# idiap/ilqr_planner

Measured on AMD Instinct MI355X. Metric: iLQR iterations/sec (7-DoF, T=200, batch 4096) + final-cost rel-err vs Eigen ref, higher is better.
Workload: dtype f64; 1 GPU; C3: PosOrn nb_deriv=1 7-DoF Panda chain, T=200, batch 4096/GPU x 1 GPU = 4096, solver=al, 20 iterations/solve, line search on, early stop off; global_batch=4096, horizon=200, parallelism=instances sharded x1, exchange=none

## Files before the change

ilqr_planner_amd/capi.py:

```python
from __future__ import annotations

import collections
import ctypes as C
import os

import numpy as np

_HERE = os.path.dirname(os.path.abspath(__file__))
LIB_PATH = os.path.join(_HERE, "libilqr_hip.so")

MAX_SEG, MAX_KP, MAX_NX, MAX_NU, MAX_NF, MAX_NQ = 24, 8, 15, 8, 15, 13
SYS_POS_ORN, SYS_POS_ORN_TIME, SYS_JOINT, SYS_JOINT_TIME = 0, 1, 2, 3
STATUS_OK, STATUS_NONFINITE, STATUS_ALPHA_FLOOR, STATUS_SWEEP_IO = 0, 1, 2, 4
LQT_MAX_NX, LQT_MAX_NU = 16, 8
CL_STATS = 5
KP_ERR, KP_STATS, CL_OUTCOME = 5, 12, 4
CL_CON_STATS, CL_OUTCOME_CON = 6, 5
KP_ERR_POS, KP_ERR_ORN, KP_ERR_VEL, KP_ERR_ANGVEL, KP_ERR_TIME = range(5)
PROF_ROLLOUT, PROF_BACKWARD, PROF_FORWARD, PROF_OTHER, PROF_APPLY = 0, 1, 2, 3, 4

EXPORTS = [
    "ilqr_dims_of", "ilqr_desc_defaults", "ilqr_ctx_create", "ilqr_ctx_destroy", "ilqr_last_error", "ilqr_ctx_set_stream",
    "ilqr_ctx_synchronize", "ilqr_version", "ilqr_problem_create", "ilqr_problem_destroy", "ilqr_problem_set_init_state",
    "ilqr_problem_set_keypoint_targets", "ilqr_problem_set_controls", "ilqr_problem_set_constraints",
# ... 282 lines not shown
        self._problems = weakref.WeakSet()
        rc = self.L.ilqr_ctx_create(device_id, C.byref(self.h))
        if rc:
            raise RuntimeError(f"ilqr_ctx_create failed (code {rc}): no usable HIP device {device_id}; there is no CPU fallback")

    def check(self, rc):
        if rc:
            raise RuntimeError(self.L.ilqr_last_error(self.h).decode())

    def set_stream(self, stream_ptr):
        self.check(self.L.ilqr_ctx_set_stream(self.h, C.c_void_p(stream_ptr)))

    def synchronize(self):
        self.check(self.L.ilqr_ctx_synchronize(self.h))

    _PINS = {"sweep": {None: 0, "mfma": 1, "rows": 2, "siwave": 4, "siwg": 5, "siwgio": 6}, "forward": {None: 0, "wg": 1, "dpp": 2, "wglds": 3}, "reroll": {None: 0, "rows": 1, "dpp": 2}}

    def set_crosscheck(self, generic_kernels=False, cp_lane_solve=False, cp_general=False, sweep=None, forward=None, reroll=None):
        pins = []
        for name, v in (("sweep", sweep), ("forward", forward), ("reroll", reroll)):
            if v not in self._PINS[name]:
                raise ValueError(f"set_crosscheck: {name} must be one of {[k for k in self._PINS[name] if k]} or None (got {v!r})")
            pins.append(self._PINS[name][v])
        self.check(self.L.ilqr_ctx_set_crosscheck(self.h, int(bool(generic_kernels)), int(bool(cp_lane_solve)), int(bool(cp_general)), *pins))

    def crosscheck_from_env(self):
        env = os.environ
        self.set_crosscheck(env.get("ILQR_HIP_PATH") == "v1", env.get("ILQR_CP_SOLVE") == "lane", env.get("ILQR_CP") == "general",
                            sweep=env.get("ILQR_SWEEP") or None, forward=env.get("ILQR_FWD") or None, reroll=env.get("ILQR_APPLY") or None)

    def set_split(self, mode: int):
# ... 433 lines not shown
```

ilqr_planner_amd/csrc/ilqr_capi.cpp:

```cpp
#include "../../include/ilqr_hip.h"

#include <hip/hip_runtime.h>

#include <cmath>
#include <cstdio>
#include <cstdlib>
#include <cstring>
#include <string>
#include <vector>

#include "ilqr_batchcp.hpp"
#include "ilqr_closed_loop.hpp"
#include "ilqr_closed_loop_cov.hpp"
#include "ilqr_ctx.hpp"
#include "ilqr_kernels.hpp"
#include "ilqr_plan.hpp"

using namespace ilqr;

struct DevScratch {
    double* ptr = nullptr;
    size_t elems = 0;
    int reserve(ilqr_ctx* c, size_t n) {
        if (elems >= n) return 0;
// ... 111 lines not shown

extern "C" int ilqr_ctx_set_stream(ilqr_ctx* c, void* s) {
    if (!c) return 1;
    c->stream = s ? (hipStream_t)s : c->own_stream;
    return 0;
}

extern "C" int ilqr_ctx_set_split(ilqr_ctx* c, int on) {
    if (!c) return 1;
    if (on < 0 || on > 2) return fail(c, "ilqr_ctx_set_split: mode must be 0, 1 or 2 (got " + std::to_string(on) + ")");
    c->split = on;
    return 0;
}

static_assert((int)SweepPin::Mfma == ILQR_XC_SWEEP_MFMA && (int)SweepPin::Rows == ILQR_XC_SWEEP_ROWS && (int)SweepPin::SiWave == ILQR_XC_SWEEP_SI_WAVE &&
              (int)SweepPin::SiWg == ILQR_XC_SWEEP_SI_WG && (int)SweepPin::SiWgIo == ILQR_XC_SWEEP_SI_WG_IO && (int)FwdPin::Wg == ILQR_XC_FWD_WG &&
              (int)FwdPin::Dpp == ILQR_XC_FWD_DPP && (int)FwdPin::WgLds == ILQR_XC_FWD_WG_LDS && (int)RerollPin::Rows == ILQR_XC_REROLL_ROWS && (int)RerollPin::Dpp == ILQR_XC_REROLL_DPP,
              "variant pins of ilqr_plan.hpp and include/ilqr_hip.h");

extern "C" int ilqr_ctx_set_crosscheck(ilqr_ctx* c, int generic_kernels, int cp_lane_solve, int cp_general, int sweep, int forward, int reroll) {
    if (!c) return 1;
    if (sweep < 0 || sweep > 6 || sweep == 3) return fail(c, "ilqr_ctx_set_crosscheck: sweep must be ILQR_XC_AUTO, ILQR_XC_SWEEP_MFMA, ILQR_XC_SWEEP_ROWS, ILQR_XC_SWEEP_SI_WAVE, ILQR_XC_SWEEP_SI_WG or ILQR_XC_SWEEP_SI_WG_IO");
    if (forward < 0 || forward > 3) return fail(c, "ilqr_ctx_set_crosscheck: forward must be ILQR_XC_AUTO, ILQR_XC_FWD_WG, ILQR_XC_FWD_DPP or ILQR_XC_FWD_WG_LDS");
    if (reroll < 0 || reroll > 2) return fail(c, "ilqr_ctx_set_crosscheck: reroll must be ILQR_XC_AUTO, ILQR_XC_REROLL_ROWS or ILQR_XC_REROLL_DPP");
    c->xc_sweep = (SweepPin)sweep;
    c->xc_forward = (FwdPin)forward;
    c->xc_reroll = (RerollPin)reroll;
    c->xc_generic = generic_kernels != 0;
    c->xc_cp_lane = cp_lane_solve != 0;
    c->xc_cp_general = cp_general != 0;
    return 0;
}

extern "C" int ilqr_ctx_synchronize(ilqr_ctx* c) {
    if (!c) return 1;
    HIPCHK(c, hipStreamSynchronize(c->stream));
    return 0;
// ... 485 lines not shown
static FwdArgs plan_fwd_args(const ilqr_problem* p, const RiccatiPlan& pl) {
    FwdArgs f;
    std::memset(&f, 0, sizeof(f));
    f.n_alpha = pl.n_alpha; f.n_kp = p->hdesc.steps.n;
    f.shared = has_shared_step(p->hdesc.steps) ? 1 : 0;
    f.n_kp_all = p->desc.n_kp;
    f.fused = pl.fused ? 1 : 0;
    f.fwd_lds = pl.fwd_lds ? 1 : 0;
    f.limits = p->desc.limits_set ? 1 : 0;
    for (int k = 0; k < p->desc.n_kp; k++) f.kp_ext |= p->desc.kp_dist[k] | p->desc.kp_has_frame[k] | p->desc.kp_has_Ru[k] | p->desc.kp_joint[k];
    return f;
}
static void launch_sweep(const ilqr_problem* p, const RiccatiPlan& pl, int h, bool al, const Bufs& bf, int B, hipStream_t st, SweepArgs& sw) {
    const int kind = p->desc.kind, nd = p->desc.nb_deriv;
    switch (pl.sweep) {
        case Sweep::SiDpp: sw.si_wg = pl.si_wg[h] ? 1 : 0; sw.si_io = pl.si_io[h] ? 1 : 0; launch_backward_si_dpp(al, pl.fused, pl.kd_sym == 1, pl.si_lanes[h], bf, B, st, sw); break;
        case Sweep::Rows: launch_backward_rows(kind, nd, al, bf, B, st); break;
        case Sweep::Mfma: launch_backward_mfma(kind, nd, al, bf, B, st); break;
        case Sweep::Generic: launch_backward_generic(kind, nd, al, bf, B, st); break;
    }
}

static int solve_riccati(ilqr_problem* p, bool al, int nb_iter, int lag, double penalty0, double scaling, int line_search, int early_stop) {
    if (!p) return 1;
    ilqr_ctx* c = p->ctx;
    if (!p->has_state || !p->has_controls) return fail(c, "set_init_state and set_controls must be called before a solve");
    if (nb_iter < 0) return fail(c, "nb_iter < 0");
    if (al && (p->bufs.m <= 0 || lag <= 0)) return fail(c, "AL solve needs constraints (ilqr_problem_set_constraints) and lag_update_step > 0");
    HIPCHK(c, hipSetDevice(c->device));
    if (ensure_trace(p, nb_iter)) return 1;
    p->last_nb_iter = nb_iter;
// ... 11 lines not shown
    FwdArgs f = plan_fwd_args(p, pl);
    f.line_search = line_search; f.early_stop = early_stop; f.nb_iter = nb_iter; f.penalty_roll = penalty0; f.al = al ? 1 : 0;
    for (int h = 0; h < nh; h++) {
        const Bufs& bf = hv[h].bufs;
        ProfScope ps(c, ILQR_PROF_ROLLOUT);
        if (pl.init == Init::Lti) launch_init_lti(kind, nd, bf, hv[h].B, hv[h].st);
        else launch_init(kind, nd, al, bf, hv[h].B, hv[h].st, penalty0);
        if (pl.init_al_update) {
            f.it = -1; f.do_update = 0;
            launch_al_update(kind, nd, bf, hv[h].B, T, hv[h].st, f);
        }
    }
    HIPCHK(c, hipGetLastError());
    double penalty = penalty0;
    SweepArgs sw;
    sw.pen_in = penalty; sw.pen_update_prev = penalty; sw.do_update_prev = 0; sw.si_wg = 0; sw.si_io = 0;
    for (int it = 0; it < nb_iter; it++) {
        FwdArgs fi = f;
        fi.it = it;
        fi.penalty_roll = penalty;
        fi.do_update = al && ((it + 1) % lag == 0);
        if (fi.do_update) penalty *= scaling;
        fi.penalty_update = penalty;
        for (int h = 0; h < nh; h++) {
            const Bufs& bf = hv[h].bufs;
            const int B = hv[h].B;
            hipStream_t st = hv[h].st;
            if (pl.split && it == 0 && h == 1) HIPCHK(c, hipStreamWaitEvent(st, c->ev_stagger, 0));
            {
                ProfScope ps(c, ILQR_PROF_OTHER);
                launch_kp_derivs(kind, nd, bf, B, st, fi);
// ... 102 lines not shown
    if (!p->has_plan)
        return fail(c, "ilqr_problem_gains needs a plan: run a solver since the problem's inputs last changed (ilqr_solve_recursive with nb_iter = 0 rolls out the controls as they are)");
    HIPCHK(c, hipSetDevice(c->device));
    const int kind = p->desc.kind, nd = p->desc.nb_deriv;
    const RiccatiPlan pl = plan_riccati(plan_input(p, false, 1, 1));
    p->has_gains = false;
    p->bufs.kd_sym = pl.kd_sym;
    if (pl.needs_ws && !p->bufs.ws)
        if (dalloc(p, &p->bufs.ws, (size_t)backward_ws_entries(kind, nd) * p->Bp, false)) return 1;
    Half hv[2];
    int nh = 1;
    if (split_begin(p, pl.split, hv, nh)) return 1;
    SplitJoin split_join{c, pl.split};
    const FwdArgs f = plan_fwd_args(p, pl);
    SweepArgs sw;
    sw.pen_in = 0.0; sw.pen_update_prev = 0.0; sw.do_update_prev = 0; sw.si_wg = 0; sw.si_io = 0;
    for (int h = 0; h < nh; h++) {
        const Bufs& bf = hv[h].bufs;
        const int B = hv[h].B;
        hipStream_t st = hv[h].st;
        {
            ProfScope ps(c, ILQR_PROF_OTHER);
            launch_gains_prepare(bf, B, st);
        }
        {
            ProfScope ps(c, ILQR_PROF_OTHER);
            launch_kp_derivs(kind, nd, bf, B, st, f);
        }
        {
            ProfScope ps(c, ILQR_PROF_BACKWARD);
            launch_sweep(p, pl, h, false, bf, B, st, sw);
// ... 536 lines not shown
```

ilqr_planner_amd/csrc/ilqr_kernels.hpp:

```cpp
#pragma once
#include <hip/hip_runtime.h>

#include "ilqr_device.hpp"
#include "ilqr_dofmap.hpp"

namespace ilqr {

struct Bufs {
    const DevDesc* desc;
    double* X[2];
    double* U[2];
    const double* U0;
    double* KD;
    const double* q0;
    const double* dq0;
    const double* kp_tg;
    double* cost;
    double* alpha;
    int* cur;
    int* active;
    int* iters;
    int* status;
    double* kpd;
    int* pend;
// ... 30 lines not shown
    int al;
    int n_alpha;
    double penalty_roll, penalty_update;
    int kp_ext;
    int limits;
    int fused;
    int fwd_lds;
};

struct SweepArgs {
    double pen_in;
    double pen_update_prev;
    int do_update_prev;
    int si_wg;
    int si_io;
};

void launch_init(int kind, int nd, bool al, const Bufs& a, int B, hipStream_t st, double penalty);
void launch_gains_prepare(const Bufs& a, int B, hipStream_t st);
void launch_kp_derivs(int kind, int nd, const Bufs& a, int B, hipStream_t st, const FwdArgs& f);
void launch_backward_generic(int kind, int nd, bool al, const Bufs& a, int B, hipStream_t st);
int backward_ws_entries(int kind, int nd);
void launch_forward_generic(int kind, int nd, bool al, const Bufs& a, int B, hipStream_t st, const FwdArgs& f);
void launch_init_lti(int kind, int nd, const Bufs& a, int B, hipStream_t st);
void launch_backward_si_dpp(bool al, bool fused, bool uniform_R, int lpi, const Bufs& a, int B, hipStream_t st, const SweepArgs& sw);
void launch_backward_rows(int kind, int nd, bool al, const Bufs& a, int B, hipStream_t st);
void launch_backward_mfma(int kind, int nd, bool al, const Bufs& a, int B, hipStream_t st);
void launch_forward_wave(int kind, bool small, const Bufs& a, int B, hipStream_t st, const FwdArgs& f);
void launch_apply_wave(int kind, const Bufs& a, int B, int T, hipStream_t st, const FwdArgs& f);
void launch_forward_lin(const Bufs& a, int B, hipStream_t st, const FwdArgs& f);
// ... 23 lines not shown
```

ilqr_planner_amd/csrc/ilqr_kernels_dpp.hip:

```cpp
#include "../../include/ilqr_hip.h"
#include "ilqr_kernels.hpp"
#include "ilqr_lanes.hpp"
#include "ilqr_step.hpp"

namespace ilqr {

namespace {

#define DPPM_ALL " row_mask:0xf bank_mask:0xf"
#define DPPM_LO " row_mask:0xf bank_mask:0x3"
#define DPPM_HI " row_mask:0xf bank_mask:0xc"


template <int LPI>
__device__ __forceinline__ void fmac_rows_all(double (&acc)[7], const double (&src)[7], const double (&mul)[7]) {
#define R_(K, LL, MASK)                                                                                                                   \
    "v_fmac_f64_dpp %[a0], %[s0], %[m" #K "] row_newbcast:" LL MASK "\n\tv_fmac_f64_dpp %[a1], %[s1], %[m" #K "] row_newbcast:" LL MASK "\n\t" \
    "v_fmac_f64_dpp %[a2], %[s2], %[m" #K "] row_newbcast:" LL MASK "\n\tv_fmac_f64_dpp %[a3], %[s3], %[m" #K "] row_newbcast:" LL MASK "\n\t" \
    "v_fmac_f64_dpp %[a4], %[s4], %[m" #K "] row_newbcast:" LL MASK "\n\tv_fmac_f64_dpp %[a5], %[s5], %[m" #K "] row_newbcast:" LL MASK "\n\t" \
    "v_fmac_f64_dpp %[a6], %[s6], %[m" #K "] row_newbcast:" LL MASK "\n\t"
#define OPS_                                                                                                                              \
    : [a0] "+v"(acc[0]), [a1] "+v"(acc[1]), [a2] "+v"(acc[2]), [a3] "+v"(acc[3]), [a4] "+v"(acc[4]), [a5] "+v"(acc[5]), [a6] "+v"(acc[6])    \
    : [s0] "v"(src[0]), [s1] "v"(src[1]), [s2] "v"(src[2]), [s3] "v"(src[3]), [s4] "v"(src[4]), [s5] "v"(src[5]), [s6] "v"(src[6]),          \
      [m0] "v"(mul[0]), [m1] "v"(mul[1]), [m2] "v"(mul[2]), [m3] "v"(mul[3]), [m4] "v"(mul[4]), [m5] "v"(mul[5]), [m6] "v"(mul[6])
// ... 67 lines not shown

__device__ __forceinline__ unsigned lds_addr(const void* p) { return (unsigned)(size_t)(const __attribute__((address_space(3))) void*)p; }
typedef __attribute__((address_space(3))) int lds_int;
__device__ __forceinline__ int flag_read(const int* p) { LDS_ORDER(); const int v = *(const lds_int*)p; LDS_ORDER(); return v; }
__device__ __forceinline__ void flag_write(int* p, int v) { LDS_ORDER(); *(lds_int*)p = v; LDS_ORDER(); }
__device__ __forceinline__ int wait_consumed(int seen, unsigned addr, int need);
__device__ __forceinline__ double ldg(const double* base, unsigned byte_off) { return *reinterpret_cast<const double*>(reinterpret_cast<const char*>(base) + byte_off); }
__device__ __forceinline__ void stg(double* base, unsigned byte_off, double v) { *reinterpret_cast<double*>(reinterpret_cast<char*>(base) + byte_off) = v; }

}

constexpr int SW_WAVES = 4;
constexpr int SW_RING = 8;
constexpr int SW_POLL_CHAIN = 1 << 20;
constexpr int SW_POLL_IO = 1 << 18;
namespace {
__device__ __forceinline__ int wait_consumed(int seen, unsigned addr, int need) {
    int v = seen, cons, cnt;
    asm volatile(
        "s_mov_b32 %[cnt], 0\n"
        "1:\n\t"
        "v_readfirstlane_b32 %[cons], %[v]\n\t"
        "s_cmp_ge_i32 %[cons], %[need]\n\t"
        "s_cbranch_scc1 2f\n\t"
        "s_cmp_ge_u32 %[cnt], %[lim]\n\t"
        "s_cbranch_scc1 2f\n\t"
        "s_sleep 1\n\t"
        "ds_read_b32 %[v], %[addr]\n\t"
        "s_add_u32 %[cnt], %[cnt], 1\n\t"
        "s_waitcnt lgkmcnt(0)\n\t"
        "s_branch 1b\n"
        "2:"
        : [v] "+v"(v), [cons] "=&s"(cons), [cnt] "=&s"(cnt)
        : [addr] "v"(addr), [need] "s"(need), [lim] "s"(SW_POLL_CHAIN)
        : "memory", "scc");
    return __builtin_amdgcn_readfirstlane(cons < need ? 1 : 0);
}
}
template <int LPI, int MR, bool FUSED, bool UNIF, bool WG = false, int IO = 0>
__global__ __launch_bounds__(WG ? (SW_WAVES + (IO ? 1 : 0)) * 64 : 64) void k_backward_si_dpp(Bufs a, SweepArgs sw) {
    constexpr int N = 7, IPW = 64 / LPI;
    constexpr int NWV = WG ? SW_WAVES : 1;
    constexpr bool IOK = (IO & 1) != 0, IOX = (IO & 2) != 0;
    constexpr int NIMG = IOK ? SW_RING : 2, XRING = SW_RING, XROW = 18;
    static_assert(!WG || (LPI == 16 && FUSED), "the workgroup form: 4 instances per wave, 16 per workgroup = one 128-byte line per row segment");
    static_assert(!IO || (WG && MR <= 1), "the I/O wave: workgroup form, at most one constraint row (256 VGPRs at two waves on a SIMD)");
    constexpr int MRR = MR > 0 ? MR : 1;
    constexpr int ROWP = kd_rowp(N), RS = UNIF ? KD_SYM_RS : N * ROWP;
    static_assert(ROWP == 8, "a gain row is the lane's eight doubles {K_r0..K_r6, d_r}");
    static_assert(LPI == 8 || LPI == 16, "");
    constexpr int NPQ_ = (IPW * (RS / 2) + 63) / 64, IMG = (IPW * RS > 128 * NPQ_) ? IPW * RS : 128 * NPQ_;
    __shared__ __attribute__((aligned(16))) double sKw[NWV][NIMG][IMG + 64];
    __shared__ double sXU[IOX ? XRING : 1][IOX ? 2 * N + 1 : 1][IOX ? XROW : 1];
    __shared__ int sFl[IO ? NWV + 1 : 1];
    const DevDesc& d = *a.desc;
    const int wv = WG ? __builtin_amdgcn_readfirstlane((int)threadIdx.x >> 6) : 0;
    double (*const sK)[IMG + 64] = sKw[wv < NWV ? wv : 0];
    const int lane = WG ? (int)threadIdx.x & 63 : (int)threadIdx.x, g = lane / LPI, l = lane % LPI;
    const int r = l & 7;
    const bool low = l < 8;
    const int b0 = (xcd_tile() * NWV + wv) * IPW;
    const int b = b0 + g;
    const int Bp = d.Bp, T = d.T;
    const bool ok = (b < d.B) && a.active[b < d.B ? b : 0];
    const int bb = (b < d.B) ? b : 0;
    const int pendw = (FUSED && b < d.B) ? a.pend[bb] : 0;
    const bool acc = pendw > 0;
    if (IO) {
        constexpr int RS_ = UNIF ? KD_SYM_RS : N * kd_rowp(N), PCS_ = RS_ / 2, NPQ2 = (IPW * PCS_ + 63) / 64;
// ... 59 lines not shown
                    Ko -= Ks;
                }
                if (IOX) {
                    if (blendi) {
                        UNR for (int q = 0; q < 4; q++) {
                            const int row = 4 * q + (lane >> 4);
                            if (row < N) stg(a.X[0], oXi + (unsigned)row * Bpi * 8u, xu[q]);
                            else if (row < 2 * N) stg(a.U[0], oXi + (unsigned)(row - N) * Bpi * 8u, xu[q]);
                        }
                    }
                    oXi -= Vs;
                }
            }
            return;
        }
        if (lane == 0) { sFl[wv] = 0; if (wv == 0) sFl[NWV] = 0; }
        __syncthreads();
    }
    if (__ballot((ok || acc) ? 1 : 0) == 0ull) return;

    const bool isV = r < N;
    const int v = isV ? r : 0;
    const int cur = a.cur[bb];
    double* const Xb = a.X[0];
    double* const Ub = a.U[0];
    const unsigned bufo = (unsigned)((a.X[1] - a.X[0]) * (ptrdiff_t)sizeof(double));
    const double aacc = acc ? ldexp(1.0, -(pendw - 1)) : 1.0;
    const bool blend = acc && pendw > 1;
    int rd = cur, r1 = blend ? 1 - cur : cur;
    if (FUSED && acc && !blend) rd = r1 = 1 - cur;
    const bool upd = FUSED && acc && sw.do_update_prev;
// ... 82 lines not shown
    constexpr int PF = 4;
    double xr[PF], ur[PF], x1r[PF], u1r[PF], lr[PF][MRR], ir[PF][MRR];
    unsigned rofs[MRR];
    UNR for (int rr = 0; rr < MRR; rr++) rofs[rr] = (unsigned)((MR > 0 && rr < m) ? rr : 0) * Bp * 8u;
    auto fetch = [&](int slot, int kk) {
        xr[slot] = ldg(Xb, oA);
        ur[slot] = ldg(Ub, oA);
        x1r[slot] = u1r[slot] = 0;
        if (FUSED) { x1r[slot] = ldg(Xb, oB); u1r[slot] = ldg(Ub, oB); }
        UNR for (int rr = 0; rr < MRR; rr++) {
            lr[slot][rr] = ir[slot][rr] = 0;
            if (MR > 0) { lr[slot][rr] = ldg(a.lambda, oL + rofs[rr]); if (!FUSED) ir[slot][rr] = ldg(a.Is, oL + rofs[rr]); }
        }
        if (kk > 0) { oA -= Vstep; oB -= Vstep; oL -= Lstep; }
    };
    UNR for (int q = 0; q < PF; q++) { fetch(q, T - 2 - q); __builtin_amdgcn_sched_barrier(0); }
    unsigned oW = (unsigned)r1 * bufo + ((unsigned)((T - 2) * N + v) * Bp + bb) * 8u;
    unsigned oLw = ((unsigned)(T - 2) * m * Bp + bb) * 8u;

    static_assert(SW_RING % PF == 0, "a step's slot is the group's first slot + its place in the group");
    const unsigned fl_cons = lds_addr(&sFl[IO ? NWV : 0]);
    int gave_up = 0;
    const int xcol = wv * IPW + g, xrow = isV ? (low ? v : N + v) : 2 * N;
    for (int k0 = T - 2; k0 >= 0; k0 -= PF) {
      const int sl0 = IOK ? (T - 2 - k0) % SW_RING : 0, xs0 = IOX ? (T - 2 - k0) % XRING : 0;
      UNR for (int jj = 0; jj < PF; jj++) {
        const int k = k0 - jj;
        double xv = ring_take(xr[jj]), uv = ring_take(ur[jj]);
        if (FUSED) {
            const double x1v = ring_take(x1r[jj]), u1v = ring_take(u1r[jj]);
            xv = fma(aacc, x1v - xv, xv);
            uv = fma(aacc, u1v - uv, uv);
        }
        double lam[MRR], Isk[MRR];
        UNR for (int rr = 0; rr < MRR; rr++) {
            lam[rr] = (MR > 0) ? ring_take(lr[jj][rr]) : 0.0;
            Isk[rr] = (MR > 0 && !FUSED) ? ring_take(ir[jj][rr]) : ir[jj][rr];
        }
        __builtin_amdgcn_sched_barrier(0);
        fetch(jj, k - PF);
        const int consumed = (IO && jj == 0) ? flag_read(&sFl[IO ? NWV : 0]) : 0;
        const bool kprev = k < T - 2;
        double kqa[NPQ], kqb[NPQ];
        if (!IOK) {
            UNR for (int q = 0; q < NPQ; q++) {
                const double2 t2 = reinterpret_cast<const double2*>(sK[(jj + 1) & 1])[lane + 64 * q];
                kqa[q] = t2.x; kqb[q] = t2.y;
            }
        }
#define SEND_()                                                                                                         \
        {                                                                                                               \
            double2* dst = reinterpret_cast<double2*>(Kout + Kstep) + lane;                                             \
            if (kfull) {                                                                                                \
                UNR for (int q = 0; q + 1 < NPQ; q++) dst[64 * q] = make_double2(kqa[q], kqb[q]);                       \
                if (lane + 64 * (NPQ - 1) < IPW * PCS) dst[64 * (NPQ - 1)] = make_double2(kqa[NPQ - 1], kqb[NPQ - 1]);  \
            } else {                                                                                                    \
                UNR for (int q = 0; q < NPQ; q++) if (pst[q]) dst[64 * q] = make_double2(kqa[q], kqb[q]);               \
            }                                                                                                           \
        }
        if (k < 0) {
            if (!IOK && k == -1) SEND_()
            continue;
        }
        if (FUSED) {
            if (IOX) sXU[xs0 + jj][xrow][xcol] = low ? xv : uv;
            else if (wr) { stg(Xb, oW, xv); stg(Ub, oW, uv); }
            oW -= Vstep;
        }
        const double Qu = Rv * uv + dt * p;
        double s[N];
        UNR for (int j = 0; j < N; j++) s[j] = fma(dt2, P[j], Dd[j]);
        double myrc = 0.0;
        pivots<LPI>(s, nm1, myrc);
        if (!IOK && kprev) SEND_()
        const double nrc = -myrc;
        double M[N], Nn[N], ntc[N], Kr[N];
        if (UNIF) {
            const double nrcD = nrc * Dj[0];
            UNR for (int j = 0; j < N; j++) {
                Nn[j] = fma(s[j], nrcD, nm1[j]);
                ntc[j] = Nn[j] * -cRN;
                Kr[j] = Nn[j] * idt;
            }
        } else {
            UNR for (int j = 0; j < N; j++) {
                M[j] = nrc * s[j];
                Nn[j] = fma(M[j], Dj[j], nm1[j]);
                ntc[j] = fma(Dv, M[j], nm1[j]) * -cRN;
                Kr[j] = Nn[j] * idt;
// ... 18 lines not shown
        if (IO) flag_write(&sFl[wv], T - 1 - k);
        Kout -= Kstep;
        double Pn[N], lx = 0;
        UNR for (int j = 0; j < N; j++) Pn[j] = -cDN * Nn[j];
        if (k == kp_next) {
            const double* src = a.kpd + (size_t)kpi * kpd_stride;
            double lxx[N];
            UNR for (int j = 0; j < N; j++) lxx[j] = AT(src, N + v * N + j, bb);
            lx = AT(src, v, bb);
            if (!isV) { UNR for (int j = 0; j < N; j++) lxx[j] = 0; lx = 0; }
            UNR for (int j = 0; j < N; j++) Pn[j] += lxx[j];
            UNR for (int j = 0; j < N; j++) asm volatile("" : "+v"(Pn[j]));
            asm volatile("" : "+v"(lx));
            kpi--;
            kp_next = (kpi >= 0) ? __builtin_amdgcn_readfirstlane(d.kp_t[kpi]) : -1;
        } else if (lim_on) {
            const double beyond = fmax(xv - smax_v, 0.0) + fmax(smin_v - xv, 0.0);
            const double lim = (beyond > 0.0) ? pen_xx : 0.0;
            if (__ballot(beyond > 0.0 ? 1 : 0) != 0ull) { UNR for (int j = 0; j < N; j++) Pn[j] = fma(-nm1[j], lim, Pn[j]); }
            lx = pen * fmax(xv - smax_v, 0.0) - pen * fmax(smin_v - xv, 0.0);
        }
        if (MR > 0) {
            UNR for (int rr = 0; rr < MRR; rr++) {
                if (MR == 1 || rr < m) {
                    const double gr = oct_row_g(Av[rr], xv, bbr[rr]);
                    if (FUSED) {
                        Isk[rr] = sw.pen_in * ((gr < 0 && lam[rr] == 0) ? 0.0 : 1.0);
                        const double nv = fma(sw.pen_update_prev, gr, lam[rr]);
                        const double nl = nv > 0 ? nv : 0;
                        lam[rr] = upd ? nl : lam[rr];
                        if (upd && l == 0) stg(a.lambda, oLw + rofs[rr], lam[rr]);
                    }
                    const double wI = Av[rr] * Isk[rr];
                    UNR for (int j = 0; j < N; j++) Pn[j] = fma(wI, Arow[rr][j], Pn[j]);
                    lx += Av[rr] * (lam[rr] + Isk[rr] * gr);
                }
            }
        }
        fmac_rows_all<LPI>(Pn, Nn, ntc);
// ... 6 lines not shown
    }
    if (IO && gave_up) {
        if (l == 0 && b < d.B) { a.active[bb] = 0; atomicOr(&a.status[bb], ILQR_STATUS_SWEEP_IO); }
        return;
    }
    if (!IOK && (T - 2) % PF == PF - 1) {
        UNR for (int q = 0; q < NPQ; q++) if (pst[q]) reinterpret_cast<double2*>(Kout + Kstep)[lane + 64 * q] = reinterpret_cast<const double2*>(sK[(PF - 1) & 1])[lane + 64 * q];
    }
    if (FUSED && acc && l == 0) {
        a.cur[bb] = 1 - cur;
        a.pend[bb] = 0;
    }
}

constexpr int SW_IO = 3;
template <int LPI, bool FUSED, bool UNIF, bool WG = false, int IO = 0>
static void launch_dpp2(bool al, const Bufs& a, int B, hipStream_t st, const SweepArgs& sw) {
    constexpr int IWG = (WG ? SW_WAVES : 1) * (64 / LPI);
    const dim3 grid(grid_x8((B + IWG - 1) / IWG)), block(WG ? (SW_WAVES + (IO ? 1 : 0)) * 64 : 64);
    if (!al || a.m == 0) hipLaunchKernelGGL((k_backward_si_dpp<LPI, 0, FUSED, UNIF, WG, IO>), grid, block, 0, st, a, sw);
    else if (a.m <= 1) hipLaunchKernelGGL((k_backward_si_dpp<LPI, 1, FUSED, UNIF, WG, IO>), grid, block, 0, st, a, sw);
    else if constexpr (IO == 0) hipLaunchKernelGGL((k_backward_si_dpp<LPI, 4, FUSED, UNIF, WG>), grid, block, 0, st, a, sw);
}

void launch_backward_si_dpp(bool al, bool fused, bool uniform_R, int lpi, const Bufs& a, int B, hipStream_t st, const SweepArgs& sw) {
    if (lpi == 16 && fused && sw.si_wg && sw.si_io && (!al || a.m <= 1)) {
        if (uniform_R) launch_dpp2<16, true, true, true, SW_IO>(al, a, B, st, sw); else launch_dpp2<16, true, false, true, SW_IO>(al, a, B, st, sw);
    } else if (lpi == 16 && fused && sw.si_wg) {
        if (uniform_R) launch_dpp2<16, true, true, true>(al, a, B, st, sw); else launch_dpp2<16, true, false, true>(al, a, B, st, sw);
    } else if (lpi == 16) {
        if (fused) { if (uniform_R) launch_dpp2<16, true, true>(al, a, B, st, sw); else launch_dpp2<16, true, false>(al, a, B, st, sw); }
        else { if (uniform_R) launch_dpp2<16, false, true>(al, a, B, st, sw); else launch_dpp2<16, false, false>(al, a, B, st, sw); }
    } else {
        if (fused) { if (uniform_R) launch_dpp2<8, true, true>(al, a, B, st, sw); else launch_dpp2<8, true, false>(al, a, B, st, sw); }
        else { if (uniform_R) launch_dpp2<8, false, true>(al, a, B, st, sw); else launch_dpp2<8, false, false>(al, a, B, st, sw); }
    }
}

}
```

ilqr_planner_amd/csrc/ilqr_plan.hpp:

```cpp
#pragma once

namespace ilqr {

constexpr int SPLIT_MIN_BATCH = 2048;
constexpr int split_first_half(int B) { return (B / 2 + 63) / 64 * 64; }


constexpr bool backward_si_supported(int kind, int nd, bool al, int m, int per_step, bool con_state_only) {
    return (kind == 0 || kind == 2) && nd == 1 && (!al || (con_state_only && per_step == 0 && m <= 4));
}
constexpr bool backward_mfma_supported(int kind, int , bool al, int m) { return kind != 2 && (!al || m <= 16); }
constexpr bool backward_rows_supported(int kind, int nd, bool al, int m) {
    return kind != 2 && !(kind == 0 && nd == 1) && (!al || m <= 16);
}
constexpr bool forward_wave_supported(int kind, int nd, int n_alpha) { return (kind == 0 || kind == 2) && nd == 1 && n_alpha <= 16; }
constexpr bool forward_lin_supported(int kind, int nd, int n_alpha) { return kind == 0 && nd == 2 && n_alpha <= 16; }
constexpr bool init_lti_supported(int kind, int nd) {
    return ((kind == 0 || kind == 1) && (nd == 1 || nd == 2)) || ((kind == 2 || kind == 3) && nd == 1);
}

inline int n_alpha_of(bool line_search, double alpha_floor) {
    int n = 1;
    if (line_search) { double a = 1.0; while (a > alpha_floor && n < 64) { a *= 0.5; n++; } }
    return n;
}

constexpr int si_lanes(int launched_B, int n_simd) { return (launched_B + 3) / 4 <= n_simd ? 16 : 8; }
constexpr int SI_WG_MIN_BATCH = 256;
constexpr int SI_IO_MIN_BATCH = 256;
constexpr bool si_io_supported(bool al, int m) { return !al || m <= 1; }

enum class SweepPin { Auto = 0, Mfma = 1, Rows = 2, SiWave = 4, SiWg = 5, SiWgIo = 6 };
enum class FwdPin { Auto = 0, Wg = 1, Dpp = 2, WgLds = 3 };
enum class RerollPin { Auto = 0, Rows = 1, Dpp = 2 };

struct PlanIn {
    int kind = 0, nd = 1;
    bool al = false;
    int m = 0, per_step = 0;
    bool con_state_only = false;
    bool limits2_set = false;
    bool shared_steps = false;
    bool uniform_R = false;
    bool off32 = true;
    bool line_search = true;
    double alpha_floor = 1e-3;
    int nb_iter = 0;
// ... 15 lines not shown
    Wave,
    WaveLast,
    Lin,
    RerollRows,
    RerollDpp,
};
constexpr int KD_SYM_KEEP = -1;

struct RiccatiPlan {
    int n_alpha = 1;
    Init init = Init::Generic;
    bool init_al_update = false;
    Sweep sweep = Sweep::Generic;
    int si_lanes[2] = {16, 16};
    bool si_wg[2] = {false, false};
    bool si_io[2] = {false, false};
    Forward forward = Forward::Generic;
    bool fwd_lds = false;
    Apply apply = Apply::None;
    bool al_update = false;
    bool fused = false;
    int kd_sym = 0;
    bool split = false;
    bool needs_ws = false;
};

inline RiccatiPlan plan_riccati(const PlanIn& in) {
    RiccatiPlan p;
    const int kind = in.kind, nd = in.nd;
    p.n_alpha = n_alpha_of(in.line_search, in.alpha_floor);
// ... 26 lines not shown
        const bool dpp = in.reroll == RerollPin::Dpp || (in.reroll == RerollPin::Auto && (in.B + 3) / 4 <= in.n_simd / 4);
        p.apply = dpp ? Apply::RerollDpp : Apply::RerollRows;
    }
    p.al_update = in.al && coop_fwd && !wave;

    p.init = cooperative && init_lti_supported(kind, nd) ? Init::Lti : Init::Generic;
    p.init_al_update = p.init == Init::Lti && in.al && !p.fused;

    p.split = coop_fwd && ((p.sweep == Sweep::Mfma && in.split) || in.split == 2) && !in.profile && in.halves && in.nb_iter > 0;
    p.needs_ws = p.sweep == Sweep::Generic && in.nb_iter > 0;
    const int b0 = p.split ? split_first_half(in.B) : in.B;
    p.si_lanes[0] = si_lanes(b0, in.n_simd);
    p.si_lanes[1] = si_lanes(in.B - b0, in.n_simd);
    const int launched[2] = {b0, in.B - b0};
    for (int h = 0; h < 2; h++) {
        const bool wg_pin = in.sweep == SweepPin::SiWg || in.sweep == SweepPin::SiWgIo;
        p.si_wg[h] = p.sweep == Sweep::SiDpp && p.si_lanes[h] == 16 && (wg_pin || (in.sweep != SweepPin::SiWave && launched[h] >= SI_WG_MIN_BATCH));
        p.si_io[h] = p.si_wg[h] && si_io_supported(in.al, in.m) &&
                     (in.sweep == SweepPin::SiWgIo || (in.sweep != SweepPin::SiWg && !p.split && launched[h] >= SI_IO_MIN_BATCH));
    }
    return p;
}

}
```

include/ilqr_hip.h:

```cpp
#ifndef ILQR_HIP_H
#define ILQR_HIP_H

#include <stddef.h>

#ifdef __cplusplus
extern "C" {
#endif

#define ILQR_MAX_SEG 24
#define ILQR_MAX_KP 8
#define ILQR_MAX_NX 15
#define ILQR_MAX_NU 8
#define ILQR_MAX_NF 15
#define ILQR_MAX_NQ 13

#define ILQR_SYS_POS_ORN 0
#define ILQR_SYS_POS_ORN_TIME 1
#define ILQR_SYS_JOINT 2
#define ILQR_SYS_JOINT_TIME 3

#define ILQR_STATUS_OK 0
#define ILQR_STATUS_NONFINITE 1
#define ILQR_STATUS_ALPHA_FLOOR 2
#define ILQR_STATUS_SWEEP_IO 4
// ... 50 lines not shown
                         const double* tool_xyz, ilqr_problem_desc* desc, double* lower, double* upper);
const char* ilqr_urdf_last_error(void);

int ilqr_ctx_create(int device_id, ilqr_ctx** out);
void ilqr_ctx_destroy(ilqr_ctx* ctx);
const char* ilqr_last_error(const ilqr_ctx* ctx);
int ilqr_ctx_set_stream(ilqr_ctx* ctx, void* hip_stream);
int ilqr_ctx_synchronize(ilqr_ctx* ctx);
int ilqr_ctx_set_split(ilqr_ctx* ctx, int on);
#define ILQR_XC_AUTO 0
#define ILQR_XC_SWEEP_MFMA 1
#define ILQR_XC_SWEEP_ROWS 2
#define ILQR_XC_SWEEP_SI_WAVE 4
#define ILQR_XC_SWEEP_SI_WG 5
#define ILQR_XC_SWEEP_SI_WG_IO 6
#define ILQR_XC_FWD_WG 1
#define ILQR_XC_FWD_DPP 2
#define ILQR_XC_FWD_WG_LDS 3
#define ILQR_XC_REROLL_ROWS 1
#define ILQR_XC_REROLL_DPP 2
int ilqr_ctx_set_crosscheck(ilqr_ctx* ctx, int generic_kernels, int cp_lane_solve, int cp_general, int sweep, int forward, int reroll);
const char* ilqr_version(void);

int ilqr_problem_create(ilqr_ctx* ctx, const ilqr_problem_desc* desc, int batch, ilqr_problem** out);
void ilqr_problem_destroy(ilqr_problem* p);

int ilqr_problem_set_init_state(ilqr_problem* p, const double* q0, const double* dq0);
int ilqr_problem_set_keypoint_targets(ilqr_problem* p, int kp_index, const double* target);
int ilqr_problem_set_controls(ilqr_problem* p, const double* U0);
int ilqr_problem_set_constraints(ilqr_problem* p, int m, int per_step, const double* A, const double* b, const double* lambda0);
// ... 137 lines not shown
```

Baseline: 13.80 million problem-iterations/s.

## Add preparing waves that precompute per-step x/u blend, limit and constraint terms for sweep

New measurement: 14.93 million problem-iterations/s, median of 6. +8.2%, better.

```diff
diff --git a/ilqr_planner_amd/capi.py b/ilqr_planner_amd/capi.py
--- a/ilqr_planner_amd/capi.py
+++ b/ilqr_planner_amd/capi.py
@@ -320,7 +320,7 @@
     def synchronize(self):
         self.check(self.L.ilqr_ctx_synchronize(self.h))
 
-    _PINS = {"sweep": {None: 0, "mfma": 1, "rows": 2, "siwave": 4, "siwg": 5, "siwgio": 6}, "forward": {None: 0, "wg": 1, "dpp": 2, "wglds": 3}, "reroll": {None: 0, "rows": 1, "dpp": 2}}
+    _PINS = {"sweep": {None: 0, "mfma": 1, "rows": 2, "siwave": 4, "siwg": 5, "siwgio": 6, "siwgprep": 7}, "forward": {None: 0, "wg": 1, "dpp": 2, "wglds": 3}, "reroll": {None: 0, "rows": 1, "dpp": 2}}
 
     def set_crosscheck(self, generic_kernels=False, cp_lane_solve=False, cp_general=False, sweep=None, forward=None, reroll=None):
         pins = []
diff --git a/ilqr_planner_amd/csrc/ilqr_capi.cpp b/ilqr_planner_amd/csrc/ilqr_capi.cpp
--- a/ilqr_planner_amd/csrc/ilqr_capi.cpp
+++ b/ilqr_planner_amd/csrc/ilqr_capi.cpp
@@ -149,13 +149,13 @@
 }
 
 static_assert((int)SweepPin::Mfma == ILQR_XC_SWEEP_MFMA && (int)SweepPin::Rows == ILQR_XC_SWEEP_ROWS && (int)SweepPin::SiWave == ILQR_XC_SWEEP_SI_WAVE &&
-              (int)SweepPin::SiWg == ILQR_XC_SWEEP_SI_WG && (int)SweepPin::SiWgIo == ILQR_XC_SWEEP_SI_WG_IO && (int)FwdPin::Wg == ILQR_XC_FWD_WG &&
+              (int)SweepPin::SiWg == ILQR_XC_SWEEP_SI_WG && (int)SweepPin::SiWgIo == ILQR_XC_SWEEP_SI_WG_IO && (int)SweepPin::SiWgPrep == ILQR_XC_SWEEP_SI_WG_PREP && (int)FwdPin::Wg == ILQR_XC_FWD_WG &&
               (int)FwdPin::Dpp == ILQR_XC_FWD_DPP && (int)FwdPin::WgLds == ILQR_XC_FWD_WG_LDS && (int)RerollPin::Rows == ILQR_XC_REROLL_ROWS && (int)RerollPin::Dpp == ILQR_XC_REROLL_DPP,
               "variant pins of ilqr_plan.hpp and include/ilqr_hip.h");
 
 extern "C" int ilqr_ctx_set_crosscheck(ilqr_ctx* c, int generic_kernels, int cp_lane_solve, int cp_general, int sweep, int forward, int reroll) {
     if (!c) return 1;
-    if (sweep < 0 || sweep > 6 || sweep == 3) return fail(c, "ilqr_ctx_set_crosscheck: sweep must be ILQR_XC_AUTO, ILQR_XC_SWEEP_MFMA, ILQR_XC_SWEEP_ROWS, ILQR_XC_SWEEP_SI_WAVE, ILQR_XC_SWEEP_SI_WG or ILQR_XC_SWEEP_SI_WG_IO");
+    if (sweep < 0 || sweep > 7 || sweep == 3) return fail(c, "ilqr_ctx_set_crosscheck: sweep must be ILQR_XC_AUTO, ILQR_XC_SWEEP_MFMA, ILQR_XC_SWEEP_ROWS, ILQR_XC_SWEEP_SI_WAVE, ILQR_XC_SWEEP_SI_WG, ILQR_XC_SWEEP_SI_WG_IO or ILQR_XC_SWEEP_SI_WG_PREP");
     if (forward < 0 || forward > 3) return fail(c, "ilqr_ctx_set_crosscheck: forward must be ILQR_XC_AUTO, ILQR_XC_FWD_WG, ILQR_XC_FWD_DPP or ILQR_XC_FWD_WG_LDS");
     if (reroll < 0 || reroll > 2) return fail(c, "ilqr_ctx_set_crosscheck: reroll must be ILQR_XC_AUTO, ILQR_XC_REROLL_ROWS or ILQR_XC_REROLL_DPP");
     c->xc_sweep = (SweepPin)sweep;
@@ -671,7 +671,7 @@
 static void launch_sweep(const ilqr_problem* p, const RiccatiPlan& pl, int h, bool al, const Bufs& bf, int B, hipStream_t st, SweepArgs& sw) {
     const int kind = p->desc.kind, nd = p->desc.nb_deriv;
     switch (pl.sweep) {
-        case Sweep::SiDpp: sw.si_wg = pl.si_wg[h] ? 1 : 0; sw.si_io = pl.si_io[h] ? 1 : 0; launch_backward_si_dpp(al, pl.fused, pl.kd_sym == 1, pl.si_lanes[h], bf, B, st, sw); break;
+        case Sweep::SiDpp: sw.si_wg = pl.si_wg[h] ? 1 : 0; sw.si_io = pl.si_io[h] ? 1 : 0; sw.si_prep = pl.si_prep[h] ? 1 : 0; launch_backward_si_dpp(al, pl.fused, pl.kd_sym == 1, pl.si_lanes[h], bf, B, st, sw); break;
         case Sweep::Rows: launch_backward_rows(kind, nd, al, bf, B, st); break;
         case Sweep::Mfma: launch_backward_mfma(kind, nd, al, bf, B, st); break;
         case Sweep::Generic: launch_backward_generic(kind, nd, al, bf, B, st); break;
@@ -713,7 +713,7 @@
     HIPCHK(c, hipGetLastError());
     double penalty = penalty0;
     SweepArgs sw;
-    sw.pen_in = penalty; sw.pen_update_prev = penalty; sw.do_update_prev = 0; sw.si_wg = 0; sw.si_io = 0;
+    sw.pen_in = penalty; sw.pen_update_prev = penalty; sw.do_update_prev = 0; sw.si_wg = 0; sw.si_io = 0; sw.si_prep = 0;
     for (int it = 0; it < nb_iter; it++) {
         FwdArgs fi = f;
         fi.it = it;
@@ -846,7 +846,7 @@
     SplitJoin split_join{c, pl.split};
     const FwdArgs f = plan_fwd_args(p, pl);
     SweepArgs sw;
-    sw.pen_in = 0.0; sw.pen_update_prev = 0.0; sw.do_update_prev = 0; sw.si_wg = 0; sw.si_io = 0;
+    sw.pen_in = 0.0; sw.pen_update_prev = 0.0; sw.do_update_prev = 0; sw.si_wg = 0; sw.si_io = 0; sw.si_prep = 0;
     for (int h = 0; h < nh; h++) {
         const Bufs& bf = hv[h].bufs;
         const int B = hv[h].B;
diff --git a/ilqr_planner_amd/csrc/ilqr_kernels.hpp b/ilqr_planner_amd/csrc/ilqr_kernels.hpp
--- a/ilqr_planner_amd/csrc/ilqr_kernels.hpp
+++ b/ilqr_planner_amd/csrc/ilqr_kernels.hpp
@@ -68,6 +68,7 @@
     int do_update_prev;
     int si_wg;
     int si_io;
+    int si_prep;
 };
 
 void launch_init(int kind, int nd, bool al, const Bufs& a, int B, hipStream_t st, double penalty);
diff --git a/ilqr_planner_amd/csrc/ilqr_kernels_dpp.hip b/ilqr_planner_amd/csrc/ilqr_kernels_dpp.hip
--- a/ilqr_planner_amd/csrc/ilqr_kernels_dpp.hip
+++ b/ilqr_planner_amd/csrc/ilqr_kernels_dpp.hip
@@ -105,6 +105,9 @@
 constexpr int SW_RING = 8;
 constexpr int SW_POLL_CHAIN = 1 << 20;
 constexpr int SW_POLL_IO = 1 << 18;
+constexpr int SW_PREP = 2;
+constexpr int SW_PRING = 8;
+constexpr int SW_PENT = 6;
 namespace {
 __device__ __forceinline__ int wait_consumed(int seen, unsigned addr, int need) {
     int v = seen, cons, cnt;
@@ -129,11 +132,13 @@
 }
 }
 template <int LPI, int MR, bool FUSED, bool UNIF, bool WG = false, int IO = 0>
-__global__ __launch_bounds__(WG ? (SW_WAVES + (IO ? 1 : 0)) * 64 : 64) void k_backward_si_dpp(Bufs a, SweepArgs sw) {
+__global__ __launch_bounds__(WG ? (SW_WAVES + (IO ? 1 : 0) + ((IO & 4) ? SW_PREP : 0)) * 64 : 64) void k_backward_si_dpp(Bufs a, SweepArgs sw) {
     constexpr int N = 7, IPW = 64 / LPI;
     constexpr int NWV = WG ? SW_WAVES : 1;
     constexpr bool IOK = (IO & 1) != 0, IOX = (IO & 2) != 0;
+    constexpr bool PRP = (IO & 4) != 0;
     constexpr int NIMG = IOK ? SW_RING : 2, XRING = SW_RING, XROW = 18;
+    static_assert(!PRP || (IOK && IOX && FUSED && SW_PRING == XRING && SW_WAVES * (64 / LPI) == 8 * SW_PREP), "the preparing waves: on top of the full I/O wave, one x | u slot per prepared slot");
     static_assert(!WG || (LPI == 16 && FUSED), "the workgroup form: 4 instances per wave, 16 per workgroup = one 128-byte line per row segment");
     static_assert(!IO || (WG && MR <= 1), "the I/O wave: workgroup form, at most one constraint row (256 VGPRs at two waves on a SIMD)");
     constexpr int MRR = MR > 0 ? MR : 1;
@@ -143,7 +148,8 @@
     constexpr int NPQ_ = (IPW * (RS / 2) + 63) / 64, IMG = (IPW * RS > 128 * NPQ_) ? IPW * RS : 128 * NPQ_;
     __shared__ __attribute__((aligned(16))) double sKw[NWV][NIMG][IMG + 64];
     __shared__ double sXU[IOX ? XRING : 1][IOX ? 2 * N + 1 : 1][IOX ? XROW : 1];
-    __shared__ int sFl[IO ? NWV + 1 : 1];
+    __shared__ __attribute__((aligned(16))) double sPr[PRP ? SW_PRING : 1][PRP ? 8 * SW_WAVES * (64 / LPI) : 1][PRP ? SW_PENT : 2];
+    __shared__ int sFl[IO ? NWV + 1 + (PRP ? SW_PREP : 0) : 1];
     const DevDesc& d = *a.desc;
     const int wv = WG ? __builtin_amdgcn_readfirstlane((int)threadIdx.x >> 6) : 0;
     double (*const sK)[IMG + 64] = sKw[wv < NWV ? wv : 0];
@@ -233,7 +239,94 @@
             }
             return;
         }
-        if (lane == 0) { sFl[wv] = 0; if (wv == 0) sFl[NWV] = 0; }
+        if (PRP && wv > NWV) {
+            const int pw = wv - NWV - 1, iw = pw * 8 + (lane >> 3), rp = lane & 7;
+            const int bi = xcd_tile() * (NWV * IPW) + iw;
+            const bool in = bi < d.B;
+            const int bbi = in ? bi : 0;
+            const bool oki = in && a.active[bbi];
+            const int pwi = in ? a.pend[bbi] : 0;
+            const int curi = a.cur[bbi];
+            __syncthreads();
+            if (__ballot((oki || pwi > 0) ? 1 : 0) == 0ull) return;
+            const bool acci = pwi > 0, blendi = pwi > 1;
+            const double aacc = acci ? ldexp(1.0, -(pwi - 1)) : 1.0;
+            int rd = curi, r1 = blendi ? 1 - curi : curi;
+            if (acci && !blendi) rd = r1 = 1 - curi;
+            const bool updi = acci && sw.do_update_prev;
+            const bool isVp = rp < N;
+            const int vp = isVp ? rp : 0;
+            const int Bpp = d.Bp, Tp = d.T;
+            const int lim_on = d.limits_set;
+            const double pen = d.penalty, pen_xx = d.pen_xx;
+            const int lw_v = isVp ? d.lw[vp] : 0;
+            const double smax_v = lw_v != 0 ? d.smax[vp] : __builtin_inf(), smin_v = lw_v != 0 ? d.smin[vp] : -__builtin_inf();
+            const double Avp = (MR == 1 && isVp) ? a.conA[vp] : 0.0, bp = (MR == 1) ? a.conb[0] : 0.0;
+            double* const Xb = a.X[0];
+            double* const Ub = a.U[0];
+            const unsigned bufo = (unsigned)((a.X[1] - a.X[0]) * (ptrdiff_t)sizeof(double));
+            const unsigned Vstep = (unsigned)N * Bpp * 8u, Lstep = (unsigned)MR * Bpp * 8u;
+            unsigned oA = (unsigned)rd * bufo + ((unsigned)((Tp - 2) * N + vp) * Bpp + bbi) * 8u;
+            unsigned oB = (unsigned)r1 * bufo + ((unsigned)((Tp - 2) * N + vp) * Bpp + bbi) * 8u;
+            unsigned oL = ((unsigned)(Tp - 2) * MR * Bpp + bbi) * 8u, oLw = oL;
+            constexpr int PF = 4;
+            double xr[PF], ur[PF], x1r[PF], u1r[PF], lr[PF];
+            auto fetch = [&](int slot, int kk) {
+                xr[slot] = ldg(Xb, oA);
+                ur[slot] = ldg(Ub, oA);
+                x1r[slot] = ldg(Xb, oB);
+                u1r[slot] = ldg(Ub, oB);
+                lr[slot] = 0;
+                if (MR > 0) lr[slot] = ldg(a.lambda, oL);
+                if (kk > 0) { oA -= Vstep; oB -= Vstep; oL -= Lstep; }
+            };
+            UNR for (int q = 0; q < PF; q++) { fetch(q, Tp - 2 - q); __builtin_amdgcn_sched_barrier(0); }
+            const unsigned fl_c = lds_addr(&sFl[NWV]);
+            int gave = 0;
+            for (int k0 = Tp - 2; k0 >= 0; k0 -= PF) {
+              const int s0 = (Tp - 2 - k0) % SW_PRING;
+              UNR for (int jj = 0; jj < PF; jj++) {
+                const int k = k0 - jj;
+                double xv = ring_take(xr[jj]), uv = ring_take(ur[jj]);
+                const double x1v = ring_take(x1r[jj]), u1v = ring_take(u1r[jj]);
+                xv = fma(aacc, x1v - xv, xv);
+                uv = fma(aacc, u1v - uv, uv);
+                double lam = (MR > 0) ? ring_take(lr[jj]) : 0.0;
+                __builtin_amdgcn_sched_barrier(0);
+                fetch(jj, k - PF);
+                if (k < 0) continue;
+                const int need = __builtin_amdgcn_readfirstlane(Tp - 1 - k - SW_PRING);
+                gave |= wait_consumed(flag_read(&sFl[NWV]), fl_c, need);
+                sXU[s0 + jj][isVp ? vp : 2 * N][iw] = xv;
+                sXU[s0 + jj][isVp ? N + vp : 2 * N][iw] = uv;
+                double beyond = 0, lim = 0, lxl = 0, Isk = 0, lt = 0;
+                if (lim_on) {
+                    beyond = fmax(xv - smax_v, 0.0) + fmax(smin_v - xv, 0.0);
+                    lim = (beyond > 0.0) ? pen_xx : 0.0;
+                    lxl = pen * fmax(xv - smax_v, 0.0) - pen * fmax(smin_v - xv, 0.0);
+                }
+                if (MR == 1) {
+                    const double gr = oct_row_g(Avp, xv, bp);
+                    Isk = sw.pen_in * ((gr < 0 && lam == 0) ? 0.0 : 1.0);
+                    const double nv = fma(sw.pen_update_prev, gr, lam);
+                    const double nl = nv > 0 ? nv : 0;
+                    lam = updi ? nl : lam;
+                    if (updi && rp == 0) stg(a.lambda, oLw, lam);
+                    lt = lam + Isk * gr;
+                    oLw -= Lstep;
+                }
+                double2* e = reinterpret_cast<double2*>(sPr[s0 + jj][iw * 8 + rp]);
+                e[0] = make_double2(uv, lim);
+                e[1] = make_double2(lxl, Isk);
+                e[2] = make_double2(lt, beyond);
+                flag_write(&sFl[NWV + 1 + pw], Tp - 1 - k);
+              }
+              k0 = gave ? 0 : k0;
+            }
+            if (gave && rp == 0 && in) { a.active[bbi] = 0; atomicOr(&a.status[bbi], ILQR_STATUS_SWEEP_IO); }
+            return;
+        }
+        if (lane == 0) { sFl[wv] = 0; if (wv == 0) { sFl[NWV] = 0; if (PRP) { UNR for (int q = 0; q < SW_PREP; q++) sFl[NWV + 1 + q] = 0; } } }
         __syncthreads();
     }
     if (__ballot((ok || acc) ? 1 : 0) == 0ull) return;
@@ -346,31 +439,38 @@
         }
         if (kk > 0) { oA -= Vstep; oB -= Vstep; oL -= Lstep; }
     };
-    UNR for (int q = 0; q < PF; q++) { fetch(q, T - 2 - q); __builtin_amdgcn_sched_barrier(0); }
+    if (!PRP) { UNR for (int q = 0; q < PF; q++) { fetch(q, T - 2 - q); __builtin_amdgcn_sched_barrier(0); } }
     unsigned oW = (unsigned)r1 * bufo + ((unsigned)((T - 2) * N + v) * Bp + bb) * 8u;
     unsigned oLw = ((unsigned)(T - 2) * m * Bp + bb) * 8u;
 
     static_assert(SW_RING % PF == 0, "a step's slot is the group's first slot + its place in the group");
     const unsigned fl_cons = lds_addr(&sFl[IO ? NWV : 0]);
+    const int fl_pi = PRP ? NWV + 1 + wv / (SW_WAVES / SW_PREP) : 0;
+    const unsigned fl_prep = lds_addr(&sFl[fl_pi]);
+    const int pent = (wv * IPW + g) * 8 + r;
     int gave_up = 0;
     const int xcol = wv * IPW + g, xrow = isV ? (low ? v : N + v) : 2 * N;
     for (int k0 = T - 2; k0 >= 0; k0 -= PF) {
       const int sl0 = IOK ? (T - 2 - k0) % SW_RING : 0, xs0 = IOX ? (T - 2 - k0) % XRING : 0;
       UNR for (int jj = 0; jj < PF; jj++) {
         const int k = k0 - jj;
-        double xv = ring_take(xr[jj]), uv = ring_take(ur[jj]);
-        if (FUSED) {
+        double xv = 0, uv = 0;
+        if (!PRP) { xv = ring_take(xr[jj]); uv = ring_take(ur[jj]); }
+        if (FUSED && !PRP) {
             const double x1v = ring_take(x1r[jj]), u1v = ring_take(u1r[jj]);
             xv = fma(aacc, x1v - xv, xv);
             uv = fma(aacc, u1v - uv, uv);
         }
         double lam[MRR], Isk[MRR];
         UNR for (int rr = 0; rr < MRR; rr++) {
-            lam[rr] = (MR > 0) ? ring_take(lr[jj][rr]) : 0.0;
-            Isk[rr] = (MR > 0 && !FUSED) ? ring_take(ir[jj][rr]) : ir[jj][rr];
-        }
-        __builtin_amdgcn_sched_barrier(0);
-        fetch(jj, k - PF);
+            lam[rr] = (MR > 0 && !PRP) ? ring_take(lr[jj][rr]) : 0.0;
+            Isk[rr] = PRP ? 0.0 : (MR > 0 && !FUSED) ? ring_take(ir[jj][rr]) : ir[jj][rr];
+        }
+        if (!PRP) {
+            __builtin_amdgcn_sched_barrier(0);
+            fetch(jj, k - PF);
+        }
+        const int prepared = (PRP && jj == 0) ? flag_read(&sFl[fl_pi]) : 0;
         const int consumed = (IO && jj == 0) ? flag_read(&sFl[IO ? NWV : 0]) : 0;
         const bool kprev = k < T - 2;
         double kqa[NPQ], kqb[NPQ];
@@ -394,17 +494,30 @@
             if (!IOK && k == -1) SEND_()
             continue;
         }
-        if (FUSED) {
+        double2 pe0 = make_double2(0, 0), pe1 = pe0, pe2 = pe0;
+#define PREP_READ_()                                                                          \
+        {                                                                                     \
+            const double2* e = reinterpret_cast<const double2*>(sPr[PRP ? sl0 + jj : 0][PRP ? pent : 0]); \
+            pe0 = e[0]; pe1 = e[1]; pe2 = e[2];                                               \
+        }
+        if (PRP && jj > 0) PREP_READ_()
+        if (FUSED && !PRP) {
             if (IOX) sXU[xs0 + jj][xrow][xcol] = low ? xv : uv;
             else if (wr) { stg(Xb, oW, xv); stg(Ub, oW, uv); }
             oW -= Vstep;
         }
-        const double Qu = Rv * uv + dt * p;
+        const double Qu0 = PRP ? 0.0 : Rv * uv + dt * p;
         double s[N];
         UNR for (int j = 0; j < N; j++) s[j] = fma(dt2, P[j], Dd[j]);
         double myrc = 0.0;
         pivots<LPI>(s, nm1, myrc);
         if (!IOK && kprev) SEND_()
+        if (PRP && jj == 0) {
+            const int last = T - 1 - k + PF - 1;
+            gave_up |= wait_consumed(prepared, fl_prep, __builtin_amdgcn_readfirstlane(last < T - 1 ? last : T - 1));
+            PREP_READ_()
+        }
+        const double Qu = PRP ? Rv * pe0.x + dt * p : Qu0;
         const double nrc = -myrc;
         double M[N], Nn[N], ntc[N], Kr[N];
         if (UNIF) {
@@ -453,6 +566,10 @@
             asm volatile("" : "+v"(lx));
             kpi--;
             kp_next = (kpi >= 0) ? __builtin_amdgcn_readfirstlane(d.kp_t[kpi]) : -1;
+        } else if (PRP && lim_on) {
+            const double lim = pe0.y;
+            if (__ballot(pe2.y > 0.0 ? 1 : 0) != 0ull) { UNR for (int j = 0; j < N; j++) Pn[j] = fma(-nm1[j], lim, Pn[j]); }
+            lx = pe1.x;
         } else if (lim_on) {
             const double beyond = fmax(xv - smax_v, 0.0) + fmax(smin_v - xv, 0.0);
             const double lim = (beyond > 0.0) ? pen_xx : 0.0;
@@ -461,7 +578,12 @@
         }
         if (MR > 0) {
             UNR for (int rr = 0; rr < MRR; rr++) {
-                if (MR == 1 || rr < m) {
+                if (PRP) {
+                    Isk[rr] = pe1.y;
+                    const double wI = Av[rr] * Isk[rr];
+                    UNR for (int j = 0; j < N; j++) Pn[j] = fma(wI, Arow[rr][j], Pn[j]);
+                    lx += Av[rr] * pe2.x;
+                } else if (MR == 1 || rr < m) {
                     const double gr = oct_row_g(Av[rr], xv, bbr[rr]);
                     if (FUSED) {
                         Isk[rr] = sw.pen_in * ((gr < 0 && lam[rr] == 0) ? 0.0 : 1.0);
@@ -498,17 +620,20 @@
 }
 
 constexpr int SW_IO = 3;
+constexpr int SW_IO_PREP = SW_IO | 4;
 template <int LPI, bool FUSED, bool UNIF, bool WG = false, int IO = 0>
 static void launch_dpp2(bool al, const Bufs& a, int B, hipStream_t st, const SweepArgs& sw) {
     constexpr int IWG = (WG ? SW_WAVES : 1) * (64 / LPI);
-    const dim3 grid(grid_x8((B + IWG - 1) / IWG)), block(WG ? (SW_WAVES + (IO ? 1 : 0)) * 64 : 64);
+    const dim3 grid(grid_x8((B + IWG - 1) / IWG)), block(WG ? (SW_WAVES + (IO ? 1 : 0) + ((IO & 4) ? SW_PREP : 0)) * 64 : 64);
     if (!al || a.m == 0) hipLaunchKernelGGL((k_backward_si_dpp<LPI, 0, FUSED, UNIF, WG, IO>), grid, block, 0, st, a, sw);
     else if (a.m <= 1) hipLaunchKernelGGL((k_backward_si_dpp<LPI, 1, FUSED, UNIF, WG, IO>), grid, block, 0, st, a, sw);
     else if constexpr (IO == 0) hipLaunchKernelGGL((k_backward_si_dpp<LPI, 4, FUSED, UNIF, WG>), grid, block, 0, st, a, sw);
 }
 
 void launch_backward_si_dpp(bool al, bool fused, bool uniform_R, int lpi, const Bufs& a, int B, hipStream_t st, const SweepArgs& sw) {
-    if (lpi == 16 && fused && sw.si_wg && sw.si_io && (!al || a.m <= 1)) {
+    if (lpi == 16 && fused && sw.si_wg && sw.si_io && sw.si_prep && (!al || a.m <= 1)) {
+        if (uniform_R) launch_dpp2<16, true, true, true, SW_IO_PREP>(al, a, B, st, sw); else launch_dpp2<16, true, false, true, SW_IO_PREP>(al, a, B, st, sw);
+    } else if (lpi == 16 && fused && sw.si_wg && sw.si_io && (!al || a.m <= 1)) {
         if (uniform_R) launch_dpp2<16, true, true, true, SW_IO>(al, a, B, st, sw); else launch_dpp2<16, true, false, true, SW_IO>(al, a, B, st, sw);
     } else if (lpi == 16 && fused && sw.si_wg) {
         if (uniform_R) launch_dpp2<16, true, true, true>(al, a, B, st, sw); else launch_dpp2<16, true, false, true>(al, a, B, st, sw);
diff --git a/ilqr_planner_amd/csrc/ilqr_plan.hpp b/ilqr_planner_amd/csrc/ilqr_plan.hpp
--- a/ilqr_planner_amd/csrc/ilqr_plan.hpp
+++ b/ilqr_planner_amd/csrc/ilqr_plan.hpp
@@ -29,8 +29,9 @@
 constexpr int SI_WG_MIN_BATCH = 256;
 constexpr int SI_IO_MIN_BATCH = 256;
 constexpr bool si_io_supported(bool al, int m) { return !al || m <= 1; }
+constexpr int SI_PREP_MIN_BATCH = 256;
 
-enum class SweepPin { Auto = 0, Mfma = 1, Rows = 2, SiWave = 4, SiWg = 5, SiWgIo = 6 };
+enum class SweepPin { Auto = 0, Mfma = 1, Rows = 2, SiWave = 4, SiWg = 5, SiWgIo = 6, SiWgPrep = 7 };
 enum class FwdPin { Auto = 0, Wg = 1, Dpp = 2, WgLds = 3 };
 enum class RerollPin { Auto = 0, Rows = 1, Dpp = 2 };
 
@@ -76,6 +77,7 @@
     Sweep sweep = Sweep::Generic;
     int si_lanes[2] = {16, 16};
     bool si_wg[2] = {false, false};
+    bool si_prep[2] = {false, false};
     bool si_io[2] = {false, false};
     Forward forward = Forward::Generic;
     bool fwd_lds = false;
@@ -132,10 +134,12 @@
     p.si_lanes[1] = si_lanes(in.B - b0, in.n_simd);
     const int launched[2] = {b0, in.B - b0};
     for (int h = 0; h < 2; h++) {
-        const bool wg_pin = in.sweep == SweepPin::SiWg || in.sweep == SweepPin::SiWgIo;
+        const bool io_pin = in.sweep == SweepPin::SiWgIo || in.sweep == SweepPin::SiWgPrep;
+        const bool wg_pin = in.sweep == SweepPin::SiWg || io_pin;
         p.si_wg[h] = p.sweep == Sweep::SiDpp && p.si_lanes[h] == 16 && (wg_pin || (in.sweep != SweepPin::SiWave && launched[h] >= SI_WG_MIN_BATCH));
         p.si_io[h] = p.si_wg[h] && si_io_supported(in.al, in.m) &&
-                     (in.sweep == SweepPin::SiWgIo || (in.sweep != SweepPin::SiWg && !p.split && launched[h] >= SI_IO_MIN_BATCH));
+                     (io_pin || (in.sweep != SweepPin::SiWg && !p.split && launched[h] >= SI_IO_MIN_BATCH));
+        p.si_prep[h] = p.si_io[h] && (in.sweep == SweepPin::SiWgPrep || (in.sweep != SweepPin::SiWgIo && launched[h] >= SI_PREP_MIN_BATCH));
     }
     return p;
 }
diff --git a/include/ilqr_hip.h b/include/ilqr_hip.h
--- a/include/ilqr_hip.h
+++ b/include/ilqr_hip.h
@@ -88,6 +88,7 @@
 #define ILQR_XC_SWEEP_SI_WAVE 4
 #define ILQR_XC_SWEEP_SI_WG 5
 #define ILQR_XC_SWEEP_SI_WG_IO 6
+#define ILQR_XC_SWEEP_SI_WG_PREP 7
 #define ILQR_XC_FWD_WG 1
 #define ILQR_XC_FWD_DPP 2
 #define ILQR_XC_FWD_WG_LDS 3
```
